# atoms-ufrj/atomsmm

Hardware: AMD Instinct MI355X
Metric: ns/day on 100k-atom TIP3P RESPA box; near-nonbonded HBM GB/s vs 8 TB/s peak (higher is better)
Workload: dtype f64

## Files before the change

atomsmm_amd/csrc/cluster.hip:

```cpp
#include <algorithm>
#include <cmath>
#include <cstdio>
#include <cstdlib>
#include <cstring>
#include <type_traits>
#include <vector>

#include "amm_ctx.h"
#include "bonded_terms.h"
#include "cluster.h"
#include "device_utils.h"
#include "pair_math.h"
#include "pair_tab.h"

#ifndef AMM_EXP_NOLJ
#define AMM_EXP_NOLJ 0
#endif

__device__ double amm_erfcx_table_dev_c[AMM_ERFCX_NI * AMM_ERFCX_NC];
static bool g_erfcx_uploaded_c[64] = {false};

void amm_cluster_classify(int n, const std::vector<int> &ptr, const std::vector<int> &idx, std::vector<int> &mol_first, std::vector<int> &rest) {
    mol_first.clear();
    rest.clear();
// ... 220 lines not shown
            aperm[3 * sl + t] = i;
            const double x = csorted_image(pos[3 * i], p0[0], sh[0], box.L[0], box.invL[0]);
            const double y = csorted_image(pos[3 * i + 1], p0[1], sh[1], box.L[1], box.invL[1]);
            const double z = csorted_image(pos[3 * i + 2], p0[2], sh[2], box.L[2], box.invL[2]);
            if (xref) {
                xref[3 * i] = pos[3 * i];
                xref[3 * i + 1] = pos[3 * i + 1];
                xref[3 * i + 2] = pos[3 * i + 2];
            }
            pf[t] = make_float4((float)x, (float)y, (float)z, 0.f);
            const float dx = pf[t].x - pf[0].x, dy = pf[t].y - pf[0].y, dz = pf[t].z - pf[0].z;
            ext2 = fmaxf(ext2, dx * dx + dy * dy + dz * dz);
            if (site_eps[i] != 0.0) sites |= 1 << t;
            if (posq_s) {
                posq_s[3 * sl + t] = make_double4(x, y, z, q[i]);
                lj_s[3 * sl + t] = make_double2(hsig[i], seps2[i]);
            }
        }
        const float ext = sqrtf(ext2) * 1.000001f + 1e-6f;
        if (!(ext <= rext)) wflags[7] = 1;
        pf[0].w = ext;
        pf[1].w = __int_as_float(sites);
        pos4f[3 * sl] = pf[0];
        pos4f[3 * sl + 1] = pf[1];
        pos4f[3 * sl + 2] = pf[2];
    }
    cbuild_tables(__builtin_amdgcn_readfirstlane(wave), lane, g, start, s_pref[threadIdx.x >> 6], tabs + wave);
}

struct CBoxF {
    float L[3], invL[3];
};

#ifndef CB_BATCH
#define CB_BATCH 5
#endif
#define CB_QCAP 256
__device__ __forceinline__ int cq_wrap(int i) { return i & (CB_QCAP - 1); }
typedef float v2f __attribute__((ext_vector_type(2)));

__device__ void cfinish_build_block(int *flags, unsigned long long *counters, const unsigned long long *blockstats, int nblocks, int count_only) {
    __shared__ unsigned long long sh_part[4][3];
    unsigned long long sum = 0, mx = 0, nr = 0;
    for (int b0 = threadIdx.x; b0 < nblocks; b0 += 8 * 256) {
        unsigned long long v[8][3];
#pragma unroll
        for (int j = 0; j < 8; ++j) {
            const int b = b0 + j * 256;
            const bool in = b < nblocks;
#pragma unroll
            for (int q = 0; q < 3; ++q) v[j][q] = in ? amm_ld_l2(&blockstats[3 * (in ? b : 0) + q]) : 0ull;
        }
#pragma unroll
        for (int j = 0; j < 8; ++j) {
            sum += v[j][0];
            mx = max(mx, v[j][1]);
            nr += v[j][2];
        }
    }
    for (int off = 32; off > 0; off >>= 1) {
        sum += __shfl_xor(sum, off);
        nr += __shfl_xor(nr, off);
        mx = max(mx, __shfl_xor(mx, off));
    }
    if ((threadIdx.x & 63) == 0) {
        sh_part[threadIdx.x >> 6][0] = sum;
        sh_part[threadIdx.x >> 6][1] = mx;
        sh_part[threadIdx.x >> 6][2] = nr;
    }
    __syncthreads();
    if (threadIdx.x == 0) {
        flags[2] = (int)max(max(sh_part[0][1], sh_part[1][1]), max(sh_part[2][1], sh_part[3][1]));
        counters[1] = sh_part[0][0] + sh_part[1][0] + sh_part[2][0] + sh_part[3][0];
        counters[2] = sh_part[0][2] + sh_part[1][2] + sh_part[2][2] + sh_part[3][2];
        if (!count_only) {
            flags[0] = 0;
            flags[AMM_FLAG_FAR] = 0;
            counters[0] += 1;
        }
    }
}

#ifndef CB_WAVES
#define CB_WAVES 5
#endif
#define CB_OCC __attribute__((amdgpu_waves_per_eu(CB_WAVES)))
#ifdef AMM_CBS_TIMING
__device__ unsigned long long g_cbs_t[8];
#define CBS_STAMP(i) do { const unsigned long long now_ = wall_clock64(); if (w == 0 && lane == 0) atomicAdd(&g_cbs_t[i], now_ - t_last); t_last = now_; } while (0)
#else
#define CBS_STAMP(i) do { } while (0)
#endif
template <bool COUNT_ONLY, bool RINT, bool SLICE = false>
__global__ void __launch_bounds__(256) __attribute__((amdgpu_waves_per_eu(SLICE ? 3 : CB_WAVES))) k_cbuild(int c_begin, int c_end, int parts, const int *__restrict__ cell_start,
                                                const float4 *__restrict__ pos4f, CBoxF box, CellGrid g, float rlist, float rnear2, int cap,
                                                int *nl, int *nnb, int *nnb_near, int *flags, unsigned long long *blockstats,
                                                unsigned long long *counters, int *ticket, int force, const int *slice_cells,
                                                const CBuildTab *__restrict__ tabs) {
    if (!force && !flags[0]) return;
    __shared__ __attribute__((aligned(16))) int s_rstart[4][128];
    __shared__ __attribute__((aligned(16))) int s_rpref[4][128];
    __shared__ float s_rshift[4][3][128];
    __shared__ int s_q[4][CB_BATCH][CB_QCAP];
    __shared__ __attribute__((aligned(16))) unsigned char s_coarse[4][CB_COARSE];
    const int lane = threadIdx.x & 63, w = threadIdx.x >> 6;
    const int wave = __builtin_amdgcn_readfirstlane((int)((blockIdx.x * blockDim.x + threadIdx.x) >> 6));
    const float FAR = 1.0e9f;
    const float rlist2 = rlist * rlist;
    unsigned long long wsum = 0, wnear = 0;
    int wmax = 0;
    const int first_cell = SLICE ? __builtin_amdgcn_readfirstlane(slice_cells[0]) : 0;
    const int nunits = SLICE ? (__builtin_amdgcn_readfirstlane(slice_cells[1]) - first_cell + 1) * parts : g.ncell * parts;
    int unit = wave;
#ifdef AMM_CBS_TIMING
    unsigned long long t_last = wall_clock64(), t_drain = 0, n_drain = 0;
#endif
    do {
    const int c = unit < nunits ? first_cell + unit / parts : g.ncell, part = unit % parts;
    int a_begin = 0, a_end = 0;
    if (c < g.ncell) {
        const int cb0 = __builtin_amdgcn_readfirstlane(cell_start[c]), cb1 = __builtin_amdgcn_readfirstlane(cell_start[c + 1]);
        const int per = (cb1 - cb0 + parts - 1) / parts;
        a_begin = max(cb0 + part * per, c_begin);
        a_end = min(min(cb0 + (part + 1) * per, cb1), c_end);
    }
    if (a_begin < a_end) {
        const CBuildTab *__restrict__ tab = tabs + c;
        const int total = __builtin_amdgcn_readfirstlane(tab->total), cshift = __builtin_amdgcn_readfirstlane(tab->cshift);
        const int4 tab_rp = reinterpret_cast<const int4 *>(tab->rstart)[lane];
        const int tab_co = reinterpret_cast<const int *>(tab->coarse)[lane];
        const int tab_code = tab->code[lane];
        const int nt0 = min(CB_BATCH, a_end - a_begin);
        float4 my = pos4f[3 * a_begin + min(lane, 3 * nt0 - 1)];
        if (lane >= 3 * nt0) my = make_float4(0.f, 0.f, 0.f, 0.f);
        *reinterpret_cast<int4 *>(lane < 32 ? &s_rstart[w][4 * lane] : &s_rpref[w][4 * (lane - 32)]) = tab_rp;
        reinterpret_cast<int *>(s_coarse[w])[lane] = tab_co;
#pragma unroll
        for (int hh = 0; hh < 2; ++hh)
#pragma unroll
            for (int k = 0; k < 3; ++k) s_rshift[w][k][lane + 64 * hh] = cshift_of((tab_code >> (8 * hh + 2 * k)) & 3, box.L[k]);
        __builtin_amdgcn_fence(__ATOMIC_RELEASE, "wavefront");
        __builtin_amdgcn_wave_barrier();
        __builtin_amdgcn_fence(__ATOMIC_ACQUIRE, "wavefront");
#ifdef AMM_CBS_TIMING
        if (SLICE && lane == 0) { atomicAdd(&g_cbs_t[7], 1ull); atomicAdd(&g_cbs_t[0], wall_clock64() - t_last); }
#endif
        for (int tb = a_begin; tb < a_end; tb += CB_BATCH) {
            const int nt = min(CB_BATCH, a_end - tb);
            if (tb > a_begin) {
                my = make_float4(0.f, 0.f, 0.f, 0.f);
                if (lane < 3 * nt) my = pos4f[3 * tb + lane];
            }
            int row_cnt = 0;
            int q_head = 0, q_cnt = 0;
            auto rl = [&](float v, int l) { return __int_as_float(__builtin_amdgcn_readlane(__float_as_int(v), l)); };
            auto drain = [&](int t, int n, auto nu_) {
                constexpr int NU = decltype(nu_)::value;
                using V = typename std::conditional<NU == 2, v2f, float>::type;
                auto pk = [](const float (&x)[NU]) -> V { if constexpr (NU == 2) return v2f{x[0], x[1]}; else return x[0]; };
                auto half = [](V x, int u) -> float { if constexpr (NU == 2) return u ? x.y : x.x; else return x; };
#ifdef AMM_CBS_TIMING
                const unsigned long long t_d0 = wall_clock64();
                n_drain++;
#endif
                const int head = __builtin_amdgcn_readlane(q_head, t);
                int slot[NU];
                bool v[NU];
                float4 A[NU][3];
#pragma unroll
                for (int u = 0; u < NU; ++u) {
                    const bool v0 = lane + 64 * u < n;
                    slot[u] = v0 ? s_q[w][t][cq_wrap(head + lane + 64 * u)] : tb + t;
                    v[u] = v0 && slot[u] != tb + t;
                }
#pragma unroll
                for (int u = 0; u < NU; ++u)
#pragma unroll
                    for (int b = 0; b < 3; ++b) A[u][b] = pos4f[3 * slot[u] + b];
                int sites[NU];
#pragma unroll
                for (int u = 0; u < NU; ++u) sites[u] = __float_as_int(A[u][1].w);
                float px[3], py[3], pz[3];
#pragma unroll
                for (int a = 0; a < 3; ++a) {
                    px[a] = rl(my.x, 3 * t + a);
                    py[a] = rl(my.y, 3 * t + a);
                    pz[a] = rl(my.z, 3 * t + a);
                }
                V ax[3], ay[3], az[3];
#pragma unroll
                for (int b = 0; b < 3; ++b) {
                    float hx[NU], hy[NU], hz[NU];
#pragma unroll
                    for (int u = 0; u < NU; ++u) {
                        hx[u] = A[u][b].x;
                        hy[u] = A[u][b].y;
                        hz[u] = A[u][b].z;
                    }
                    ax[b] = pk(hx);
                    ay[b] = pk(hy);
                    az[b] = pk(hz);
                }
                if (!RINT) {
                    const V sx = box.L[0] * __builtin_elementwise_rint((ax[0] - px[0]) * box.invL[0]);
                    const V sy = box.L[1] * __builtin_elementwise_rint((ay[0] - py[0]) * box.invL[1]);
                    const V sz = box.L[2] * __builtin_elementwise_rint((az[0] - pz[0]) * box.invL[2]);
#pragma unroll
                    for (int b = 0; b < 3; ++b) {
                        ax[b] -= sx;
                        ay[b] -= sy;
                        az[b] -= sz;
                    }
                }
                V m2;
                if constexpr (NU == 2) m2 = v2f{3.0e38f, 3.0e38f};
                else m2 = 3.0e38f;
#pragma unroll
                for (int a = 0; a < 3; ++a)
#pragma unroll
                    for (int b = 0; b < 3; ++b) {
                        V dx = px[a] - ax[b], dy = py[a] - ay[b], dz = pz[a] - az[b];
                        if (RINT) {
                            dx -= box.L[0] * __builtin_elementwise_rint(dx * box.invL[0]);
                            dy -= box.L[1] * __builtin_elementwise_rint(dy * box.invL[1]);
                            dz -= box.L[2] * __builtin_elementwise_rint(dz * box.invL[2]);
                        }
                        V r2 = dx * dx;
                        r2 = __builtin_elementwise_fma(dy, dy, r2);
                        r2 = __builtin_elementwise_fma(dz, dz, r2);
                        m2 = __builtin_elementwise_min(m2, r2);
                    }
#pragma unroll
                for (int u = 0; u < NU; ++u) {
                    const float m2u = half(m2, u);
                    const bool pass = v[u] && m2u < rlist2;
                    const unsigned long long m_pass = __builtin_amdgcn_ballot_w64(pass);
                    if (m_pass != 0ull) {
                        const bool is_near = pass && m2u < rnear2;
                        const unsigned long long m_near = __builtin_amdgcn_ballot_w64(is_near);
                        const int np_ = __popcll(m_pass), nn_ = __popcll(m_near);
                        const int c2 = __builtin_amdgcn_readlane(row_cnt, t);
                        const int cnt = c2 & 0xffff, cntf = (int)((unsigned)c2 >> 16);
                        if (!COUNT_ONLY) {
                            const int mp = __builtin_amdgcn_mbcnt_hi((unsigned)(m_pass >> 32), __builtin_amdgcn_mbcnt_lo((unsigned)m_pass, 0u));
                            const int mn = __builtin_amdgcn_mbcnt_hi((unsigned)(m_near >> 32), __builtin_amdgcn_mbcnt_lo((unsigned)m_near, 0u));
                            const int pos_near = cnt + mn, pos_far = (cap - 1 - cntf) - (mp - mn);
                            if (cnt + cntf + np_ <= cap) {
                                int *row_out = nl + (size_t)(tb + t - c_begin) * cap;
                                if (pass) row_out[is_near ? pos_near : pos_far] = slot[u] | (sites[u] << 29);
                            }
                        }
                        row_cnt = lane == t ? c2 + nn_ + ((np_ - nn_) << 16) : row_cnt;
                    }
                }
                q_head = lane == t ? cq_wrap(head + n) : q_head;
                q_cnt = lane == t ? q_cnt - n : q_cnt;
#ifdef AMM_CBS_TIMING
                t_drain += wall_clock64() - t_d0;
#endif
            };
            auto fetch = [&](int cb, float4 (&cand)[2], int (&js)[2]) {
#pragma unroll
                for (int u = 0; u < 2; ++u) {
                    const int idx = cb + u * 64 + lane;
                    const bool in = idx < total;
                    int r = s_coarse[w][idx >> cshift];
                    while (r < 127 && s_rpref[w][r + 1] <= idx) ++r;
                    const int slot = in ? s_rstart[w][r] + idx - s_rpref[w][r] : 0;
                    float4 q = pos4f[3 * slot];
                    if (!RINT) {
                        const float sx = s_rshift[w][0][r], sy = s_rshift[w][1][r], sz = s_rshift[w][2][r];
                        q.x = in ? q.x + sx : FAR;
                        q.y = in ? q.y + sy : FAR;
                        q.z = in ? q.z + sz : FAR;
                    } else if (!in) {
                        q.w = -1.0e9f;
                    }
                    cand[u] = q;
                    js[u] = slot;
                }
            };
            float4 cand[2], cand_n[2];
            int js[2], js_n[2];
            fetch(0, cand, js);
            const float plim_l = my.w + rlist;
            for (int cb = 0; cb < total; cb += 128) {
                if (cb + 128 < total) fetch(cb + 128, cand_n, js_n);
                const v2f cx = v2f{cand[0].x, cand[1].x}, cy = v2f{cand[0].y, cand[1].y}, cz = v2f{cand[0].z, cand[1].z};
                const v2f cw = v2f{cand[0].w, cand[1].w};
                for (int t = 0; t < nt; ++t) {
                    const float p0x = rl(my.x, 3 * t), p0y = rl(my.y, 3 * t), p0z = rl(my.z, 3 * t), plim = rl(plim_l, 3 * t);
                    int qn = __builtin_amdgcn_readlane(q_cnt, t);
                    const int head = __builtin_amdgcn_readlane(q_head, t);
                    v2f dx = p0x - cx, dy = p0y - cy, dz = p0z - cz;
                    if (RINT) {
                        dx -= box.L[0] * __builtin_elementwise_rint(dx * box.invL[0]);
                        dy -= box.L[1] * __builtin_elementwise_rint(dy * box.invL[1]);
                        dz -= box.L[2] * __builtin_elementwise_rint(dz * box.invL[2]);
                    }
                    v2f r2 = dx * dx;
                    r2 = __builtin_elementwise_fma(dy, dy, r2);
                    r2 = __builtin_elementwise_fma(dz, dz, r2);
                    const v2f lim = plim + cw;
                    const v2f lim2 = lim * lim;
#pragma unroll
                    for (int u = 0; u < 2; ++u) {
                        const bool pass = (u ? r2.y < lim2.y : r2.x < lim2.x) && (!RINT || (u ? lim.y : lim.x) > 0.f);
                        const unsigned long long m = __builtin_amdgcn_ballot_w64(pass);
                        if (m == 0ull) continue;
                        const int at = qn + __builtin_amdgcn_mbcnt_hi((unsigned)(m >> 32), __builtin_amdgcn_mbcnt_lo((unsigned)m, 0u));
                        if (pass) s_q[w][t][cq_wrap(head + at)] = js[u];
                        qn += __popcll(m);
                    }
                    q_cnt = lane == t ? qn : q_cnt;
                    if (qn >= 128) {
                        __builtin_amdgcn_fence(__ATOMIC_RELEASE, "wavefront");
                        __builtin_amdgcn_wave_barrier();
                        __builtin_amdgcn_fence(__ATOMIC_ACQUIRE, "wavefront");
                        drain(t, 128, std::integral_constant<int, 2>());
                    }
                }
#pragma unroll
                for (int u = 0; u < 2; ++u) {
                    cand[u] = cand_n[u];
                    js[u] = js_n[u];
                }
            }
            __builtin_amdgcn_fence(__ATOMIC_RELEASE, "wavefront");
            __builtin_amdgcn_wave_barrier();
            __builtin_amdgcn_fence(__ATOMIC_ACQUIRE, "wavefront");
            for (int t = 0; t < nt; ++t) {
                const int n = __builtin_amdgcn_readlane(q_cnt, t);
#if CB_HALF_DRAIN
                if (n > 64) drain(t, n, std::integral_constant<int, 2>());
                else if (n > 0) drain(t, n, std::integral_constant<int, 1>());
#else
                if (n > 0) drain(t, n, std::integral_constant<int, 2>());
#endif
            }
            __builtin_amdgcn_fence(__ATOMIC_RELEASE, "wavefront");
            __builtin_amdgcn_wave_barrier();
            if (lane < nt) {
                const int count = row_cnt & 0xffff, countf = (int)((unsigned)row_cnt >> 16);
                const int total_nb = count + countf;
                if (!COUNT_ONLY) {
                    const bool over = total_nb > cap;
                    nnb[tb + lane - c_begin] = over ? 0 : total_nb;
                    nnb_near[tb + lane - c_begin] = over ? 0 : count;
                    if (over) flags[1] = 1;
                }
                wsum += (unsigned long long)total_nb;
                wnear += (unsigned long long)count;
                wmax = max(wmax, total_nb);
            }
        }
    }
#ifdef AMM_CBS_TIMING
    if (SLICE && lane == 0 && a_begin < a_end) { atomicAdd(&g_cbs_t[1], wall_clock64() - t_last); atomicAdd(&g_cbs_t[2], t_drain); atomicAdd(&g_cbs_t[3], n_drain); }
#endif
    unit += (int)(gridDim.x * (blockDim.x >> 6));
    } while (SLICE && unit < nunits);
    for (int off = 32; off > 0; off >>= 1) {
        wsum += __shfl_xor(wsum, off);
        wnear += __shfl_xor(wnear, off);
        wmax = max(wmax, __shfl_xor(wmax, off));
    }
    __shared__ unsigned long long s_sum[4], s_near[4];
    __shared__ int s_max[4];
    if (lane == 0) {
        s_sum[w] = wsum;
        s_near[w] = wnear;
        s_max[w] = wmax;
    }
    __syncthreads();
    if (threadIdx.x == 0) {
        amm_st_l2(&blockstats[3 * blockIdx.x], s_sum[0] + s_sum[1] + s_sum[2] + s_sum[3]);
        amm_st_l2(&blockstats[3 * blockIdx.x + 1], (unsigned long long)max(max(s_max[0], s_max[1]), max(s_max[2], s_max[3])));
        amm_st_l2(&blockstats[3 * blockIdx.x + 2], s_near[0] + s_near[1] + s_near[2] + s_near[3]);
    }
    if (amm_last_block(ticket)) cfinish_build_block(flags, counters, blockstats, (int)gridDim.x, COUNT_ONLY ? 1 : 0);
}

#ifndef CBS_BATCH
#define CBS_BATCH 3
#endif
#ifndef CBS_SEG
#define CBS_SEG 384
#endif
#define CBS_MAXCH (4 * CBS_SEG / 128)
template <bool RINT>
__global__ void __launch_bounds__(256) k_cbuild_split(int c_begin, int c_end, int parts, const int *__restrict__ cell_start,
                                                      const float4 *__restrict__ pos4f, CBoxF box, CellGrid g, float rlist, float rnear2, int cap,
                                                      int *nl, int *nnb, int *nnb_near, int *flags, unsigned long long *blockstats,
                                                      unsigned long long *counters, int *ticket, int force, const int *slice_cells) {
    if (!force && !flags[0]) return;
    __shared__ int s_rstart[128];
    __shared__ int s_rpref[128];
    __shared__ float s_rshift[3][128];
    __shared__ unsigned char s_coarse[CB_COARSE];
    __shared__ int s_total;
    __shared__ int s_ring[4][CBS_BATCH][CBS_SEG];
    __shared__ int s_cnt[4][CBS_BATCH];
    __shared__ int s_stage[CBS_BATCH * CBS_MAXCH][128];
    __shared__ int s_ccnt[CBS_BATCH * CBS_MAXCH];
    const int lane = threadIdx.x & 63, w = threadIdx.x >> 6;
    const float FAR = 1.0e9f;
    const float rlist2 = rlist * rlist;
    unsigned long long wsum = 0, wnear = 0;
    int wmax = 0;
    const int first_cell = __builtin_amdgcn_readfirstlane(slice_cells[0]);
    const int nunits = (__builtin_amdgcn_readfirstlane(slice_cells[1]) - first_cell + 1) * parts;
    for (int unit = (int)blockIdx.x; unit < nunits; unit += (int)gridDim.x) {
    const int c = first_cell + unit / parts, part = unit % parts;
    int a_begin = 0, a_end = 0;
    if (c < g.ncell) {
        const int cb0 = __builtin_amdgcn_readfirstlane(cell_start[c]), cb1 = __builtin_amdgcn_readfirstlane(cell_start[c + 1]);
        const int per = (cb1 - cb0 + parts - 1) / parts;
        a_begin = max(cb0 + part * per, c_begin);
        a_end = min(min(cb0 + (part + 1) * per, cb1), c_end);
    }
    if (a_begin < a_end) {
#ifdef AMM_CBS_TIMING
        unsigned long long t_last = wall_clock64();
        if (w == 0 && lane == 0) atomicAdd(&g_cbs_t[7], 1ull);
#endif
        const int ncx = g.nc[0], ncy = g.nc[1], ncz = g.nc[2];
        const int cx = c % ncx, cy = (c / ncx) % ncy, cz = c / (ncx * ncy);
        if (w == 0) {
            const int nsx = g.nstencil[0], nsy = g.nstencil[1], ne = nsx * nsy * g.nstencil[2];
            int ecs[2] = {0, 0}, len[2] = {0, 0}, inc[2];
            float esx[2] = {0.f, 0.f}, esy[2] = {0.f, 0.f}, esz[2] = {0.f, 0.f};
#pragma unroll
            for (int hh = 0; hh < 2; ++hh) {
                const int e = lane + 64 * hh;
                if (e < ne) {
                    const int ox = e % nsx, oy = (e / nsx) % nsy, oz = e / (nsx * nsy);
                    int nz = ncz < 2 * g.h[2] + 1 ? oz : cz - g.h[2] + oz;
                    esz[hh] = nz < 0 ? -box.L[2] : (nz >= ncz ? box.L[2] : 0.f);
                    nz = nz < 0 ? nz + ncz : (nz >= ncz ? nz - ncz : nz);
                    int ny = ncy < 2 * g.h[1] + 1 ? oy : cy - g.h[1] + oy;
                    esy[hh] = ny < 0 ? -box.L[1] : (ny >= ncy ? box.L[1] : 0.f);
                    ny = ny < 0 ? ny + ncy : (ny >= ncy ? ny - ncy : ny);
                    int nx = ncx < 2 * g.h[0] + 1 ? ox : cx - g.h[0] + ox;
                    esx[hh] = nx < 0 ? -box.L[0] : (nx >= ncx ? box.L[0] : 0.f);
                    nx = nx < 0 ? nx + ncx : (nx >= ncx ? nx - ncx : nx);
                    const int cc = (nz * ncy + ny) * ncx + nx;
                    ecs[hh] = cell_start[cc];
                    len[hh] = cell_start[cc + 1] - ecs[hh];
                }
                inc[hh] = len[hh];
                for (int off = 1; off < 64; off <<= 1) {
                    const int v = __shfl_up(inc[hh], off);
                    if (lane >= off) inc[hh] += v;
                }
            }
            const int lower = __builtin_amdgcn_readlane(inc[0], 63);
            if (lane == 0) s_total = lower + __builtin_amdgcn_readlane(inc[1], 63);
#pragma unroll
            for (int hh = 0; hh < 2; ++hh) {
                s_rstart[lane + 64 * hh] = ecs[hh];
                s_rpref[lane + 64 * hh] = (hh ? lower : 0) + inc[hh] - len[hh];
                s_rshift[0][lane + 64 * hh] = esx[hh];
                s_rshift[1][lane + 64 * hh] = esy[hh];
                s_rshift[2][lane + 64 * hh] = esz[hh];
            }
        }
        __syncthreads();
        const int total = s_total;
        int cshift = 3;
        while (((total + 127) >> cshift) > CB_COARSE) ++cshift;
        {
            const int idx = (int)threadIdx.x << cshift;
            int r = 0;
#pragma unroll
            for (int step = 64; step > 0; step >>= 1)
                if (s_rpref[r + step] <= idx) r += step;
            s_coarse[threadIdx.x] = (unsigned char)r;
        }
        __syncthreads();
        CBS_STAMP(0);
        const int rounds = (total + 4 * CBS_SEG - 1) / (4 * CBS_SEG);
        const int seg = (((total + rounds - 1) / rounds + 511) >> 9) << 7;
        auto rl = [&](float v, int l) { return __int_as_float(__builtin_amdgcn_readlane(__float_as_int(v), l)); };
        for (int tb = a_begin; tb < a_end; tb += CBS_BATCH) {
            const int nt = min(CBS_BATCH, a_end - tb);
            float4 my = make_float4(0.f, 0.f, 0.f, 0.f);
            if (lane < 3 * nt) my = pos4f[3 * tb + lane];
            const float plim_l = my.w + rlist;
            int row_cnt = 0;
            for (int r0 = 0; r0 < total; r0 += 4 * seg) {
// ... 1964 lines not shown
```

atomsmm_amd/csrc/pair.hip:

```cpp
#include <atomic>
#include <cmath>
#include <cstdio>
#include <cstdlib>
#include <cstring>

#include "amm_ctx.h"
#include "bonded_terms.h"
#include "cluster.h"
#include "device_utils.h"
#include "pair_args.h"
#include "pair_math.h"
#include "pair_tab.h"

int amm_pair_build_consts(const amm_pair_desc &d, PairConsts &pc) {
    pc.family = d.family;
    pc.flags = d.flags;
    pc.degree = d.degree < 1 ? 1 : d.degree;
    pc.cmode = (d.flags & AMM_COULOMB_EWALD) ? 1 : ((d.flags & AMM_COULOMB_RF) ? 2 : 0);
    pc.sign = d.sign;
    pc.rc = d.rc;
    pc.rc2 = d.rc * d.rc;
    pc.rc0 = d.rc0;
    pc.rs0 = d.rs0;
    pc.inv_dr0 = (d.rc0 > d.rs0) ? 1.0 / (d.rc0 - d.rs0) : 0.0;
// ... 1810 lines not shown
            if (pf->desc.family == AMM_DAMPED && pf->pc.degree == 1) rc_ = launch_pair_dual<AMM_DAMPED, 1>(grid, block, st, guest->desc.family, A, pf->pc, guest->pc);
            else if (pf->desc.family == AMM_DAMPED) rc_ = launch_pair_dual<AMM_DAMPED, 0>(grid, block, st, guest->desc.family, A, pf->pc, guest->pc);
            else if (pf->desc.family == AMM_NONBONDED && pf->pc.cmode == 1)
                rc_ = launch_pair_dual<AMM_NONBONDED, 1>(grid, block, st, guest->desc.family, A, pf->pc, guest->pc);
            else if (pf->desc.family == AMM_NONBONDED && pf->pc.cmode == 2)
                rc_ = launch_pair_dual<AMM_NONBONDED, 2>(grid, block, st, guest->desc.family, A, pf->pc, guest->pc);
            else if (pf->desc.family == AMM_NONBONDED)
                rc_ = launch_pair_dual<AMM_NONBONDED, 0>(grid, block, st, guest->desc.family, A, pf->pc, guest->pc);
            else {
                amm_set_error("dual evaluation: unsupported host family");
                rc_ = 1;
            }
            if (rc_) return 1;
            guest->n_evals++;
            guest->last_fused = 1;
        } else if (pf->pc.flags & (AMM_GROUP_LJ | AMM_GROUP_Q)) {
            if (pf->desc.family == AMM_NEAR_FSWITCH) launch_pair_grouped<AMM_NEAR_FSWITCH>(grid, block, st, guard, en, A, pf->pc);
            else if (pf->desc.family == AMM_NONBONDED && pf->pc.cmode == 0) launch_pair_grouped<AMM_NONBONDED>(grid, block, st, false, en, A, pf->pc);
            else {
                amm_set_error("interaction groups (AMM_GROUP_LJ / AMM_GROUP_Q) are supported for the NEAR_FSWITCH and plain NONBONDED families");
                return 1;
            }
        } else
        switch (pf->desc.family) {
        case AMM_NEAR_NONE: launch_pair<AMM_NEAR_NONE, 0>(grid, block, st, guard, en, A, pf->pc); break;
        case AMM_NEAR_SHIFT: launch_pair<AMM_NEAR_SHIFT, 0>(grid, block, st, guard, en, A, pf->pc); break;
        case AMM_NEAR_FSWITCH: launch_pair<AMM_NEAR_FSWITCH, 0>(grid, block, st, guard, en, A, pf->pc); break;
        case AMM_DAMPED:
            if (pf->pc.degree == 1) launch_pair<AMM_DAMPED, 1>(grid, block, st, false, en, A, pf->pc);
            else launch_pair<AMM_DAMPED, 0>(grid, block, st, false, en, A, pf->pc);
            break;
        case AMM_SOFTCORE:
            if (pf->d_lambda_dev) {
                amm_set_error("softcore force with lambda on the device evaluated through its neighbour list: call amm_pair_set_lambda first");
                return 1;
            }
            launch_pair<AMM_SOFTCORE, 0>(grid, block, st, false, en, A, pf->pc);
            break;
        case AMM_LJ_VIRIAL: launch_pair<AMM_LJ_VIRIAL, 0>(grid, block, st, false, en, A, pf->pc); break;
        case AMM_PAIR_EXPR:
            if (amm_pair_expr_launch(ctx, pf, A, grid, en)) return 1;
            break;
        case AMM_NONBONDED:
            if (pf->pc.cmode == 1) launch_pair<AMM_NONBONDED, 1>(grid, block, st, false, en, A, pf->pc);
            else if (pf->pc.cmode == 2) launch_pair<AMM_NONBONDED, 2>(grid, block, st, false, en, A, pf->pc);
            else launch_pair<AMM_NONBONDED, 0>(grid, block, st, false, en, A, pf->pc);
            break;
        default: amm_set_error("unknown pair family"); return 1;
        }
        if (timed) AMM_HIP(hipEventRecord(e1, st));
        AMM_HIP(hipGetLastError());
        if (en) {
            if (amm_reduce_add(ctx, pf->d_epart, nblk, 1.0, d_energy)) return 1;
        }
    }
    pf->n_evals++;
    if (exchange) {
        PendingExchange &pe = ctx->pending;
        pe.active = true;
        pe.per = per;
        pe.nf = nf;
        pe.perm = L->d_perm;
        pe.force = d_force;
        pe.gforce = g_force;
        if (ctx->comm) {
            if (amm_comm_allgather_impl(ctx, ctx->d_xchg, (size_t)nf * per * 3)) return 1;
            if (amm_exchange_finish_impl(ctx)) return 1;
        }
    }
    return 0;
}

bool amm_pair_can_eval_dual(amm_ctx *ctx, PairForce *guest, PairForce *host) {
    if (!guest || !host || guest->host != host || host->host) return false;
    if (guest->dual_ok >= 0) return guest->dual_ok == 1;
    guest->dual_ok = 0;
    const int gf = guest->desc.family, hf = host->desc.family;
    if (!(gf == AMM_NEAR_NONE || gf == AMM_NEAR_SHIFT || gf == AMM_NEAR_FSWITCH)) return false;
    if (!(hf == AMM_DAMPED || hf == AMM_NONBONDED)) return false;
    if ((guest->desc.flags & AMM_GUARD_RC0) || (host->desc.flags & AMM_GUARD_RC0)) return false;
    if ((guest->desc.flags | host->desc.flags) & (AMM_GROUP_LJ | AMM_GROUP_Q)) return false;
    if (!(guest->desc.rc <= host->desc.rc)) return false;
    if (guest->pc.Kc != host->pc.Kc) return false;
    const size_t n = (size_t)ctx->n;
    std::vector<double> a(n), b(n);
    const double *ga[3] = {guest->d_q, guest->d_hsig, guest->d_seps2}, *ha[3] = {host->d_q, host->d_hsig, host->d_seps2};
    for (int k = 0; k < 3; ++k) {
        if (hipMemcpy(a.data(), ga[k], sizeof(double) * n, hipMemcpyDeviceToHost) != hipSuccess) return false;
        if (hipMemcpy(b.data(), ha[k], sizeof(double) * n, hipMemcpyDeviceToHost) != hipSuccess) return false;
        if (std::memcmp(a.data(), b.data(), sizeof(double) * n) != 0) return false;
    }
    guest->dual_ok = 1;
    return true;
}

__global__ void __launch_bounds__(256) k_count_within(PairArgs A, double r2w, int nslice, unsigned long long *out) {
    const int tid = blockIdx.x * blockDim.x + threadIdx.x;
    const int a = tid >> A.lpa_shift, sub = tid & ((1 << A.lpa_shift) - 1);
    unsigned long long cnt = 0;
    if (a < nslice) {
        const int s = A.s_begin + a;
        const double4 pi = A.posq_s[s];
        const int nfront = A.nnb[a], nn = A.nnb_total ? A.nnb_total[a] : nfront;
        const int *row = A.nl + (size_t)a * A.cap;
        const int back = A.cap - 1 + nfront;
        for (int k = sub; k < nn; k += 1 << A.lpa_shift) {
            const double4 pj = A.posq_s[row[k < nfront ? k : back - k]];
            const double dx = amm_min_image(pi.x - pj.x, A.box.L[0], A.box.invL[0]);
            const double dy = amm_min_image(pi.y - pj.y, A.box.L[1], A.box.invL[1]);
            const double dz = amm_min_image(pi.z - pj.z, A.box.L[2], A.box.invL[2]);
            cnt += (dx * dx + dy * dy + dz * dz < r2w) ? 1ull : 0ull;
        }
    }
    for (int off = 32; off > 0; off >>= 1) cnt += __shfl_xor(cnt, off);
    if ((threadIdx.x & 63) == 0 && cnt) atomicAdd(out, cnt);
}

int amm_pair_count_within_impl(amm_ctx *ctx, PairForce *pf, const double *d_pos, double r_within, long long *count) {
    PairForce *L = pf->host ? pf->host : pf;
    if (!L->built) {
        amm_set_error("amm_pair_count_within: evaluate the force once first (the neighbour rows do not exist yet)");
        return 1;
    }
    hipStream_t st = ctx->stream;
    const int n = pf->n;
    hipLaunchKernelGGL(k_gather_sorted, dim3((n + 255) / 256), dim3(256), 0, st, n, L->d_perm, d_pos, pf->d_q, pf->d_hsig,
                       pf->d_seps2, ctx->box, pf->d_posq_s, pf->d_lj_s);
    PairArgs A;
    std::memset(&A, 0, sizeof(A));
    A.s_begin = L->s_begin;
    A.s_end = L->s_end;
    A.lpa_shift = 3;
    A.cap = L->cap;
    A.nl = L->d_nl;
    A.nnb = L->d_nnb_near;
    A.nnb_total = (pf == L && L->rnear_build > 0) ? L->d_nnb : nullptr;
    A.posq_s = pf->d_posq_s;
    A.box = ctx->box;
    const int nslice = L->s_end - L->s_begin;
    unsigned long long *d_cnt = L->d_counters + 7;
    AMM_HIP(hipMemsetAsync(d_cnt, 0, sizeof(unsigned long long), st));
    if (nslice > 0)
        hipLaunchKernelGGL(k_count_within, dim3((unsigned)(((long)nslice * 8 + 255) / 256)), dim3(256), 0, st, A, r_within * r_within, nslice, d_cnt);
    unsigned long long h = 0;
    AMM_HIP(hipMemcpyAsync(&h, d_cnt, sizeof(h), hipMemcpyDeviceToHost, st));
    AMM_HIP(hipStreamSynchronize(st));
    *count = (long long)h;
    return 0;
}

extern "C" __attribute__((weak)) const char *amm_variant_tag(void);
const char *amm_kernel_revision_impl() {
#ifdef AMM_CLUSTER_TUNE
    return "r10-lookupoffset-tune";
#else
    return amm_variant_tag ? "r10-lookupoffset-tune" : "r10-lookupoffset";
#endif
}

int amm_pair_table_check_impl(const amm_pair_desc &d, double site_sigma, double site_eps, double site_q, long long out[8]) {
    PairConsts pc;
    if (amm_pair_build_consts(d, pc)) return 1;
    std::vector<double> coef;
    SiteTable ss;
    ss.want = site_eps > 0.0 && site_sigma > 0.0 && site_q != 0.0;
    ss.sig = site_sigma;
    ss.eps4 = 4.0 * site_eps;
    ss.QQ = pc.Kc * site_q * site_q;
    amm_build_coulomb_table(pc, coef, &ss);
    if (ss.coef.empty()) pc.tab.ss_first = -1;
    const TabIndexCheck R = amm_tab_indices_in_range(pc.tab, amm_tab_pass_rc2(pc));
    out[0] = pc.tab.nint;
    out[1] = pc.tab.ss_first;
    out[2] = R.points;
    out[3] = R.bad;
    out[4] = R.idx_min;
    out[5] = R.idx_max;
    out[6] = pc.tab.nA;
    out[7] = AMM_TAB_SHIFT - pc.tab.shiftB;
    return 0;
}

int amm_pair_build_table(PairForce *pf) {
    std::vector<double> coef;
    SiteTable ss;
    ss.want = pf->cluster_ok && pf->one_site_class && pf->site_one_charge && pf->site_q != 0.0 && pf->site_seps2 != 0.0;
    ss.sig = 2.0 * pf->site_hsig;
    ss.eps4 = pf->site_seps2 * pf->site_seps2;
    ss.QQ = pf->pc.Kc * pf->site_q * pf->site_q;
    pf->tab_error = amm_build_coulomb_table(pf->pc, coef, &ss);
    pf->ss_built_for[0] = pf->site_hsig;
    pf->ss_built_for[1] = pf->site_seps2;
    pf->ss_built_for[2] = ss.want ? pf->site_q : 0.0;
    if (pf->d_tab) {
        (void)hipFree(pf->d_tab);
        pf->d_tab = nullptr;
    }
    if (pf->d_tab_ss) {
        (void)hipFree(pf->d_tab_ss);
        pf->d_tab_ss = nullptr;
    }
    pf->ss_error = ss.error;
    static std::atomic<unsigned long long> uploads{0};
    pf->tab_serial = ++uploads;
    if (pf->pc.tab.nint > 0 && !(pf->tab_error <= AMM_TAB_MAX_ERROR)) {
        pf->pc.tab.nint = 0;
        coef.clear();
    }
    if (pf->pc.tab.nint > 0 && amm_tab_indices_in_range(pf->pc.tab, amm_tab_pass_rc2(pf->pc)).bad != 0) {
        pf->pc.tab.nint = 0;
        coef.clear();
    }
    if (pf->pc.tab.nint == 0 || ss.coef.empty() || !(ss.error <= AMM_TAB_SS_MAX_ERROR)) {
        pf->pc.tab.ss_first = -1;
        ss.coef.clear();
    }
    if (pf->pc.tab.nint > 0) {
        AMM_HIP(hipMalloc(&pf->d_tab, sizeof(double) * coef.size()));
        AMM_HIP(hipMemcpy(pf->d_tab, coef.data(), sizeof(double) * coef.size(), hipMemcpyHostToDevice));
    }
    if (!ss.coef.empty()) {
        AMM_HIP(hipMalloc(&pf->d_tab_ss, sizeof(double) * ss.coef.size()));
        AMM_HIP(hipMemcpy(pf->d_tab_ss, ss.coef.data(), sizeof(double) * ss.coef.size(), hipMemcpyHostToDevice));
    }
    return 0;
}

bool amm_pair_can_fuse_discount(amm_ctx *ctx, PairForce *guest, PairForce *host) {
    if (!guest || !host || guest->host != host || host->host) return false;
    if (!(guest->desc.flags & AMM_GUARD_RC0)) return false;
    if (guest->fuse_ok >= 0) return guest->fuse_ok == 1;
    guest->fuse_ok = 0;
    if (!ctx->opt_tab) return false;
    const int gf = guest->desc.family, hf = host->desc.family;
    if (!(gf == AMM_NEAR_NONE || gf == AMM_NEAR_SHIFT || gf == AMM_NEAR_FSWITCH)) return false;
    if (!(hf == AMM_DAMPED || hf == AMM_NONBONDED)) return false;
    if ((host->desc.flags & AMM_GUARD_RC0) || host->pc.sign != 1.0) return false;
    if ((guest->desc.flags | host->desc.flags) & (AMM_GROUP_LJ | AMM_GROUP_Q)) return false;
    if (!(guest->pc.tab.nint > 0 && guest->d_tab && host->pc.tab.nint > 0 && host->d_tab)) return false;
    if (guest->pc.Kc != host->pc.Kc) return false;
    const size_t n = (size_t)ctx->n;
    std::vector<double> a(n), b(n);
    const double *ga[3] = {guest->d_q, guest->d_hsig, guest->d_seps2}, *ha[3] = {host->d_q, host->d_hsig, host->d_seps2};
    for (int k = 0; k < 3; ++k) {
        if (hipMemcpy(a.data(), ga[k], sizeof(double) * n, hipMemcpyDeviceToHost) != hipSuccess) return false;
        if (hipMemcpy(b.data(), ha[k], sizeof(double) * n, hipMemcpyDeviceToHost) != hipSuccess) return false;
        if (std::memcmp(a.data(), b.data(), sizeof(double) * n) != 0) return false;
    }
    guest->fuse_ok = 1;
    return true;
}

int amm_pair_free(PairForce *pf) {
    void *ptrs[] = {pf->d_q, pf->d_hsig, pf->d_seps2, pf->d_excl_ptr, pf->d_excl_idx, pf->d_cell_of, pf->d_cell_count,
                    pf->d_cell_start, pf->d_cell_members, pf->d_perm, pf->d_posq_s, pf->d_lj_s, pf->d_xref,
                    pf->d_nl, pf->d_nnb, pf->d_flags, pf->d_counters, pf->d_epart, pf->d_pos4f_s, pf->d_blockstats, pf->d_inv_perm, pf->d_nnb_near, pf->d_nl_out, pf->d_nnb_out,
                    pf->d_nnb_scratch, pf->d_xref_out, pf->d_ticket, pf->d_tab, pf->d_cls, pf->d_cell_count_lj, pf->d_cell_start_lj,
                    pf->d_row_order, pf->d_member, pf->d_active, pf->d_cell_sets, pf->d_nnb_lj, pf->d_mol_first, pf->d_rest_idx};
    for (void *p : ptrs)
        if (p) (void)hipFree(p);
    for (PairForce::TabImage &im : pf->tab_image)
        if (im.d) (void)hipFree(im.d);
    for (hipEvent_t e : pf->ev) (void)hipEventDestroy(e);
    if (pf->cl) amm_cluster_free(pf->cl);
    if (pf->small) amm_small_group_free(pf->small);
    amm_pair_expr_free(pf->expr);
    delete pf;
    return 0;
}

int amm_pair_setup_grid(amm_ctx *ctx, PairForce *pf) { return setup_grid(ctx, pf); }

int amm_pair_regrid(amm_ctx *ctx, PairForce *pf) {
    void **owned[] = {(void **)&pf->d_nnb, (void **)&pf->d_nnb_near, (void **)&pf->d_nnb_out, (void **)&pf->d_nnb_scratch, (void **)&pf->d_row_order,
                      (void **)&pf->d_nnb_lj, (void **)&pf->d_active, (void **)&pf->d_cell_members, (void **)&pf->d_cell_sets, (void **)&pf->d_blockstats,
                      (void **)&pf->d_nl_out, (void **)&pf->d_nl};
    for (void **p : owned) {
        if (*p) (void)hipFree(*p);
        *p = nullptr;
    }
    pf->built = false;
    pf->capc = pf->cap = pf->cap_out = 0;
    pf->active_cap = pf->active_size = 0;
    pf->built_rows = 0;
    if (setup_grid(ctx, pf)) return 1;
    const int nc = pf->grid.ncell;
    if (nc > pf->ncell_alloc) {
        for (int **p : {&pf->d_cell_count, &pf->d_cell_start, &pf->d_cell_count_lj, &pf->d_cell_start_lj}) {
            if (*p) (void)hipFree(*p);
            *p = nullptr;
            AMM_HIP(hipMalloc(p, sizeof(int) * (nc + 1)));
        }
        pf->ncell_alloc = nc;
    }
    AMM_HIP(hipMemset(pf->d_cell_count, 0, sizeof(int) * (nc + 1)));
    AMM_HIP(hipMemset(pf->d_cell_count_lj, 0, sizeof(int) * (nc + 1)));
    AMM_HIP(hipMemset(pf->d_flags, 0, sizeof(int) * 16));
    AMM_HIP(hipMemset(pf->d_ticket, 0, sizeof(int) * 4 * AMM_TICKET_INTS));
    return 0;
}
```

Before: 1207.

## Restructure cluster neighbor-list build loops with scalar-held row state and batched drains

Reworks the cluster neighbor-list build so per-row queue heads and counts sit in unrolled scalar arrays and a bitmask, instead of being read back per lane with readlane. Row positions and box constants are hoisted out of the candidate loop and pinned in SGPRs through empty asm constraints. Queue drains are batched: all full rows are collected into a pending mask and drained after a single barrier per candidate block, not one barrier per row. The drain routine now keeps its row count in a scalar and resolves the self-pair test through ballots. This aims to cut readlane/VALU overhead and synchronization in the build kernel, at the cost of more SGPR pressure and the risk of sgpr spills or changed unrolling.

```diff
diff --git a/atomsmm_amd/csrc/cluster.hip b/atomsmm_amd/csrc/cluster.hip
--- a/atomsmm_amd/csrc/cluster.hip
+++ b/atomsmm_amd/csrc/cluster.hip
@@ -396,9 +396,9 @@
                 if (lane < 3 * nt) my = pos4f[3 * tb + lane];
             }
             int row_cnt = 0;
-            int q_head = 0, q_cnt = 0;
+            v2f b_x = v2f{box.L[0], box.invL[0]}, b_y = v2f{box.L[1], box.invL[1]}, b_z = v2f{box.L[2], box.invL[2]};
             auto rl = [&](float v, int l) { return __int_as_float(__builtin_amdgcn_readlane(__float_as_int(v), l)); };
-            auto drain = [&](int t, int n, auto nu_) {
+            auto drain = [&](int t, int n, int head, auto nu_) {
                 constexpr int NU = decltype(nu_)::value;
                 using V = typename std::conditional<NU == 2, v2f, float>::type;
                 auto pk = [](const float (&x)[NU]) -> V { if constexpr (NU == 2) return v2f{x[0], x[1]}; else return x[0]; };
@@ -407,16 +407,12 @@
                 const unsigned long long t_d0 = wall_clock64();
                 n_drain++;
 #endif
-                const int head = __builtin_amdgcn_readlane(q_head, t);
+                const int self = tb + t;
                 int slot[NU];
-                bool v[NU];
                 float4 A[NU][3];
 #pragma unroll
-                for (int u = 0; u < NU; ++u) {
-                    const bool v0 = lane + 64 * u < n;
-                    slot[u] = v0 ? s_q[w][t][cq_wrap(head + lane + 64 * u)] : tb + t;
-                    v[u] = v0 && slot[u] != tb + t;
-                }
+                for (int u = 0; u < NU; ++u)
+                    slot[u] = lane + 64 * u < n ? s_q[w][t][cq_wrap(head + lane + 64 * u)] : self;
 #pragma unroll
                 for (int u = 0; u < NU; ++u)
 #pragma unroll
@@ -445,10 +441,13 @@
                     ay[b] = pk(hy);
                     az[b] = pk(hz);
                 }
+                asm volatile("" : "+s"(b_x), "+s"(b_y), "+s"(b_z));
+                auto edge = [](const v2f &b) -> V { if constexpr (NU == 2) return b.xx; else return b.x; };
+                auto inv = [](const v2f &b) -> V { if constexpr (NU == 2) return b.yy; else return b.y; };
                 if (!RINT) {
-                    const V sx = box.L[0] * __builtin_elementwise_rint((ax[0] - px[0]) * box.invL[0]);
-                    const V sy = box.L[1] * __builtin_elementwise_rint((ay[0] - py[0]) * box.invL[1]);
-                    const V sz = box.L[2] * __builtin_elementwise_rint((az[0] - pz[0]) * box.invL[2]);
+                    const V sx = edge(b_x) * __builtin_elementwise_rint((ax[0] - px[0]) * inv(b_x));
+                    const V sy = edge(b_y) * __builtin_elementwise_rint((ay[0] - py[0]) * inv(b_y));
+                    const V sz = edge(b_z) * __builtin_elementwise_rint((az[0] - pz[0]) * inv(b_z));
 #pragma unroll
                     for (int b = 0; b < 3; ++b) {
                         ax[b] -= sx;
@@ -465,40 +464,39 @@
                     for (int b = 0; b < 3; ++b) {
                         V dx = px[a] - ax[b], dy = py[a] - ay[b], dz = pz[a] - az[b];
                         if (RINT) {
-                            dx -= box.L[0] * __builtin_elementwise_rint(dx * box.invL[0]);
-                            dy -= box.L[1] * __builtin_elementwise_rint(dy * box.invL[1]);
-                            dz -= box.L[2] * __builtin_elementwise_rint(dz * box.invL[2]);
+                            dx -= edge(b_x) * __builtin_elementwise_rint(dx * inv(b_x));
+                            dy -= edge(b_y) * __builtin_elementwise_rint(dy * inv(b_y));
+                            dz -= edge(b_z) * __builtin_elementwise_rint(dz * inv(b_z));
                         }
                         V r2 = dx * dx;
                         r2 = __builtin_elementwise_fma(dy, dy, r2);
                         r2 = __builtin_elementwise_fma(dz, dz, r2);
                         m2 = __builtin_elementwise_min(m2, r2);
                     }
+                int c2 = __builtin_amdgcn_readlane(row_cnt, t);
+                char *row_out = reinterpret_cast<char *>(nl + (size_t)(self - c_begin) * cap);
 #pragma unroll
                 for (int u = 0; u < NU; ++u) {
                     const float m2u = half(m2, u);
-                    const bool pass = v[u] && m2u < rlist2;
-                    const unsigned long long m_pass = __builtin_amdgcn_ballot_w64(pass);
+                    const bool other = slot[u] != self, in_list = m2u < rlist2, in_near = m2u < rnear2;
+                    const unsigned long long m_pass = __builtin_amdgcn_ballot_w64(other) & __builtin_amdgcn_ballot_w64(in_list);
                     if (m_pass != 0ull) {
-                        const bool is_near = pass && m2u < rnear2;
-                        const unsigned long long m_near = __builtin_amdgcn_ballot_w64(is_near);
+                        const unsigned long long m_near = m_pass & __builtin_amdgcn_ballot_w64(in_near);
                         const int np_ = __popcll(m_pass), nn_ = __popcll(m_near);
-                        const int c2 = __builtin_amdgcn_readlane(row_cnt, t);
                         const int cnt = c2 & 0xffff, cntf = (int)((unsigned)c2 >> 16);
                         if (!COUNT_ONLY) {
                             const int mp = __builtin_amdgcn_mbcnt_hi((unsigned)(m_pass >> 32), __builtin_amdgcn_mbcnt_lo((unsigned)m_pass, 0u));
                             const int mn = __builtin_amdgcn_mbcnt_hi((unsigned)(m_near >> 32), __builtin_amdgcn_mbcnt_lo((unsigned)m_near, 0u));
                             const int pos_near = cnt + mn, pos_far = (cap - 1 - cntf) - (mp - mn);
                             if (cnt + cntf + np_ <= cap) {
-                                int *row_out = nl + (size_t)(tb + t - c_begin) * cap;
-                                if (pass) row_out[is_near ? pos_near : pos_far] = slot[u] | (sites[u] << 29);
+                                const unsigned at = (unsigned)(in_near ? pos_near : pos_far) << 2;
+                                if (other && in_list) *reinterpret_cast<int *>(row_out + at) = slot[u] | (sites[u] << 29);
                             }
                         }
-                        row_cnt = lane == t ? c2 + nn_ + ((np_ - nn_) << 16) : row_cnt;
+                        c2 += nn_ + ((np_ - nn_) << 16);
                     }
                 }
-                q_head = lane == t ? cq_wrap(head + n) : q_head;
-                q_cnt = lane == t ? q_cnt - n : q_cnt;
+                row_cnt = lane == t ? c2 : row_cnt;
 #ifdef AMM_CBS_TIMING
                 t_drain += wall_clock64() - t_d0;
 #endif
@@ -528,41 +526,66 @@
             int js[2], js_n[2];
             fetch(0, cand, js);
             const float plim_l = my.w + rlist;
+            v2f r_xy[CB_BATCH], r_zl[CB_BATCH];
+            int r_qn[CB_BATCH];
+#pragma unroll
+            for (int t = 0; t < CB_BATCH; ++t) {
+                r_xy[t] = v2f{rl(my.x, 3 * t), rl(my.y, 3 * t)};
+                r_zl[t] = v2f{rl(my.z, 3 * t), rl(plim_l, 3 * t)};
+                r_qn[t] = 0;
+            }
+            unsigned r_head = 0;
             for (int cb = 0; cb < total; cb += 128) {
                 if (cb + 128 < total) fetch(cb + 128, cand_n, js_n);
                 const v2f cx = v2f{cand[0].x, cand[1].x}, cy = v2f{cand[0].y, cand[1].y}, cz = v2f{cand[0].z, cand[1].z};
                 const v2f cw = v2f{cand[0].w, cand[1].w};
-                for (int t = 0; t < nt; ++t) {
-                    const float p0x = rl(my.x, 3 * t), p0y = rl(my.y, 3 * t), p0z = rl(my.z, 3 * t), plim = rl(plim_l, 3 * t);
-                    int qn = __builtin_amdgcn_readlane(q_cnt, t);
-                    const int head = __builtin_amdgcn_readlane(q_head, t);
-                    v2f dx = p0x - cx, dy = p0y - cy, dz = p0z - cz;
+                unsigned pend = 0;
+                int rows = nt;
+                asm volatile("" : "+s"(rows));
+#pragma unroll
+                for (int t = 0; t < CB_BATCH; ++t) {
+                    if (t >= rows) break;
+                    int qn = r_qn[t];
+                    const int head = (int)((r_head >> t) & 1u) << 7;
+                    if (!SLICE) asm volatile("" : "+s"(r_xy[t]), "+s"(r_zl[t]));
+                    const v2f xy = SLICE ? v2f{rl(my.x, 3 * t), rl(my.y, 3 * t)} : r_xy[t], zl = SLICE ? v2f{rl(my.z, 3 * t), rl(plim_l, 3 * t)} : r_zl[t];
+                    v2f dx = xy.xx - cx, dy = xy.yy - cy, dz = zl.xx - cz;
                     if (RINT) {
-                        dx -= box.L[0] * __builtin_elementwise_rint(dx * box.invL[0]);
-                        dy -= box.L[1] * __builtin_elementwise_rint(dy * box.invL[1]);
-                        dz -= box.L[2] * __builtin_elementwise_rint(dz * box.invL[2]);
+                        asm volatile("" : "+s"(b_x), "+s"(b_y), "+s"(b_z));
+                        dx -= b_x.xx * __builtin_elementwise_rint(dx * b_x.yy);
+                        dy -= b_y.xx * __builtin_elementwise_rint(dy * b_y.yy);
+                        dz -= b_z.xx * __builtin_elementwise_rint(dz * b_z.yy);
                     }
                     v2f r2 = dx * dx;
                     r2 = __builtin_elementwise_fma(dy, dy, r2);
                     r2 = __builtin_elementwise_fma(dz, dz, r2);
-                    const v2f lim = plim + cw;
+                    const v2f lim = zl.yy + cw;
                     const v2f lim2 = lim * lim;
 #pragma unroll
                     for (int u = 0; u < 2; ++u) {
                         const bool pass = (u ? r2.y < lim2.y : r2.x < lim2.x) && (!RINT || (u ? lim.y : lim.x) > 0.f);
                         const unsigned long long m = __builtin_amdgcn_ballot_w64(pass);
                         if (m == 0ull) continue;
-                        const int at = qn + __builtin_amdgcn_mbcnt_hi((unsigned)(m >> 32), __builtin_amdgcn_mbcnt_lo((unsigned)m, 0u));
-                        if (pass) s_q[w][t][cq_wrap(head + at)] = js[u];
+                        const int at = __builtin_amdgcn_mbcnt_hi((unsigned)(m >> 32), __builtin_amdgcn_mbcnt_lo((unsigned)m, 0u)) + (head + qn);
+                        if (pass) s_q[w][t][cq_wrap(at)] = js[u];
                         qn += __popcll(m);
                     }
-                    q_cnt = lane == t ? qn : q_cnt;
-                    if (qn >= 128) {
-                        __builtin_amdgcn_fence(__ATOMIC_RELEASE, "wavefront");
-                        __builtin_amdgcn_wave_barrier();
-                        __builtin_amdgcn_fence(__ATOMIC_ACQUIRE, "wavefront");
-                        drain(t, 128, std::integral_constant<int, 2>());
-                    }
+                    r_qn[t] = qn;
+                    pend |= qn >= 128 ? 1u << t : 0u;
+                }
+                if (pend) {
+                    __builtin_amdgcn_fence(__ATOMIC_RELEASE, "wavefront");
+                    __builtin_amdgcn_wave_barrier();
+                    __builtin_amdgcn_fence(__ATOMIC_ACQUIRE, "wavefront");
+                    unsigned todo = pend;
+                    do {
+                        const int t = __builtin_ctz(todo);
+                        todo &= todo - 1;
+                        drain(t, 128, (int)((r_head >> t) & 1u) << 7, std::integral_constant<int, 2>());
+                    } while (todo);
+                    r_head ^= pend;
+#pragma unroll
+                    for (int t = 0; t < CB_BATCH; ++t) r_qn[t] &= 127;
                 }
 #pragma unroll
                 for (int u = 0; u < 2; ++u) {
@@ -573,13 +596,17 @@
             __builtin_amdgcn_fence(__ATOMIC_RELEASE, "wavefront");
             __builtin_amdgcn_wave_barrier();
             __builtin_amdgcn_fence(__ATOMIC_ACQUIRE, "wavefront");
+#pragma unroll 1
             for (int t = 0; t < nt; ++t) {
-                const int n = __builtin_amdgcn_readlane(q_cnt, t);
+                int n = 0;
+#pragma unroll
+                for (int k = 0; k < CB_BATCH; ++k) n = k == t ? r_qn[k] : n;
+                const int head = (int)((r_head >> t) & 1u) << 7;
 #if CB_HALF_DRAIN
-                if (n > 64) drain(t, n, std::integral_constant<int, 2>());
-                else if (n > 0) drain(t, n, std::integral_constant<int, 1>());
+                if (n > 64) drain(t, n, head, std::integral_constant<int, 2>());
+                else if (n > 0) drain(t, n, head, std::integral_constant<int, 1>());
 #else
-                if (n > 0) drain(t, n, std::integral_constant<int, 2>());
+                if (n > 0) drain(t, n, head, std::integral_constant<int, 2>());
 #endif
             }
             __builtin_amdgcn_fence(__ATOMIC_RELEASE, "wavefront");
diff --git a/atomsmm_amd/csrc/pair.hip b/atomsmm_amd/csrc/pair.hip
--- a/atomsmm_amd/csrc/pair.hip
+++ b/atomsmm_amd/csrc/pair.hip
@@ -1986,9 +1986,9 @@
 extern "C" __attribute__((weak)) const char *amm_variant_tag(void);
 const char *amm_kernel_revision_impl() {
 #ifdef AMM_CLUSTER_TUNE
-    return "r10-lookupoffset-tune";
+    return "r11-buildloops-tune";
 #else
-    return amm_variant_tag ? "r10-lookupoffset-tune" : "r10-lookupoffset";
+    return amm_variant_tag ? "r11-buildloops-tune" : "r11-buildloops";
 #endif
 }
 
```

Result: faster. 1235 (median of 6 runs) (+2.3%).
